# keyber/Single-Image-Super-Resolution

Hardware: AMD Instinct MI355X
Metric: HR patches/sec (x2 generator fwd+bwd, LR 96x96 -> SR 192x192) (higher is better)
Workload: dtype f32; 1 GPU; SRGAN x2 generator (16 blocks, 64 features, spectral norm) fwd+bwd+Adam with bicubic LR degradation and pixel-MSE x10, per-GPU batch 16 HR 192x192 patches (LR 96x96 -> SR 192x192): the north star's headline. BASELINE.json's metric string "96^2 crops, x4" is configs.cfg3 of this line. Single build: fp32.; per_gpu_batch=16, hr=192, lr=96, parallelism=dp1, hip_graph=True

## Files before the change

include/sisr_hip.h:

```cpp
#ifndef SISR_HIP_H
#define SISR_HIP_H

#include <stdint.h>

#ifdef __cplusplus
extern "C" {
#endif

#define SISR_E_BADARG (-1)
#define SISR_E_TOOBIG (-2)
#define SISR_E_UNSUPPORTED (-3)

enum {
    SISR_PRO_NONE = 0,
    SISR_PRO_ACT = 1,
    SISR_PRO_AFFINE_ACT = 2,
    SISR_PRO_BNBWD = 3,
    SISR_PRO_BNACT_BWD = 4,
    SISR_PRO_ACT_BWD = 5,
    SISR_PRO_TANH_BWD = 6,
    SISR_PRO_RES_AFFINE = 7
};
enum { SISR_X_NHWC = 0, SISR_X_NCHW = 1, SISR_X_NHWC_UNSHUFFLE2 = 2 };
enum { SISR_Y_NHWC = 0, SISR_Y_NCHW = 1, SISR_Y_NHWC_SHUFFLE2 = 2 };
// ... 67 lines not shown

typedef struct SisrWgradDeepPlan {
    int32_t enabled;
    int32_t TH, TW, tiles_x, tiles_q, n_tiles;
    int32_t PR;
    int32_t IW, IH_max;
    int32_t IWd, IHd_max;
    int32_t NPOS_max;
    int32_t XP_max;
    int32_t NITX, NITD;
    int32_t n_pb, tiles_per_pb;
    int32_t n_cib, n_cob;
    int32_t lds_bytes;
    int32_t slab_bf16;
    int32_t batch_first_wg;
    uint32_t m_tiles_x, m_tw, m_ho, m_pr, m_iw, m_iwd;
} SisrWgradDeepPlan;

typedef struct SisrWgradDesc {
    const float *x1, *x2, *pa, *pb, *pd, *ps, *pt;
    const float *g1, *g2, *qa, *qb, *qd, *qs, *qt;
    float *slab;
    float *bias_slab;
    int32_t N, H, W, Cin, Ho, Wo, Cout;
    int32_t KH, KW, stride, pad_y, pad_x;
    int32_t x_mode, pro_mode;
    const float *pro_slope_p;
    float pro_slope;
    int32_t g_mode, gpro_mode;
    const float *gpro_slope_p;
    float gpro_slope;
    int32_t TH, TW, TN, tiles_y, tiles_x, n_groups, n_tiles;
    int32_t CK, PS, KROWP, n_chunk, CoutPad;
    int32_t NJ, NP, NT, TSTEP, TVALID;
    int32_t grid_x, n_slabs, slab_elems, lds_bytes;
    uint32_t m_tiles_x, m_tiles_y, m_iw, m_twp, m_kw;
    int32_t x_bf16, g_bf16;
    int32_t mfma_split;
    int64_t slab_stride;
    SisrWgradDeepPlan deep;
} SisrWgradDesc;

int sisr_wgrad_plan(SisrWgradDesc *d, int32_t max_pixel_blocks);
int sisr_conv2d_plan_bf16(SisrConvDesc *d);
int sisr_conv2d_bf16(const SisrConvDesc *d, void *stream);
int sisr_conv2d_deep_plan(SisrConvDesc *d, int32_t target_wg, int32_t prefer_bn, int32_t classes);
int sisr_conv2d_deep_eligible(const SisrConvDesc *d);
int sisr_conv2d_trunk_eligible(const SisrConvDesc *d);
int sisr_conv2d_bf16_parts(const SisrConvDesc *d);
int sisr_conv2d_trunk_f32_eligible(const SisrConvDesc *d);
int sisr_conv2d_f32_parts(const SisrConvDesc *d);
int sisr_conv2d_f32_bnb_parts(const SisrConvDesc *d);
int sisr_conv2d_thin_eligible(const SisrConvDesc *d);
int sisr_conv2d_toimage_eligible(const SisrConvDesc *d);
int sisr_conv2d_toimage_f32_eligible(const SisrConvDesc *d);
int sisr_wgrad_plan_bf16(SisrWgradDesc *d, int32_t max_pixel_blocks);
int sisr_wgrad_deep_plan(SisrWgradDesc *d, int32_t target_wg);
int sisr_wgrad_deep_eligible(const SisrWgradDesc *d);
int sisr_wgrad_deep_batch(const SisrWgradDesc *table_host, const SisrWgradDesc *table_dev, int32_t n, void *stream);
int sisr_wgrad_trunk_batch_arg_bytes(void);
int sisr_wgrad_trunk_batch_args(const SisrWgradDesc *descs, int32_t n, void *args_host);
int sisr_wgrad_trunk_batch(const SisrWgradDesc *descs, const void *args_dev, int32_t n, int32_t wgs_per_layer, void *stream);
int sisr_wgrad_trunk_f32_batch_arg_bytes(void);
int sisr_wgrad_trunk_f32_batch_args(const SisrWgradDesc *descs, int32_t n, void *args_host);
int sisr_wgrad_trunk_f32_batch(const SisrWgradDesc *descs, const void *args_dev, int32_t n, int32_t wgs_per_layer, void *stream);
int sisr_conv2d_wgrad_bf16(const SisrWgradDesc *d, void *stream);
int sisr_wgrad_trunk_eligible(const SisrWgradDesc *d);
int sisr_wgrad_bf16_slabs(const SisrWgradDesc *d);
int sisr_wgrad_trunk_f32_eligible(const SisrWgradDesc *d);
int sisr_wgrad_f32_slabs(const SisrWgradDesc *d);
int sisr_wgrad_thin_eligible(const SisrWgradDesc *d);
int sisr_wgrad_toimage_eligible(const SisrWgradDesc *d);
int sisr_wgrad_toimage_f32_eligible(const SisrWgradDesc *d);
int sisr_conv2d_wgrad_f32(const SisrWgradDesc *d, void *stream);
int sisr_slab_reduce_f32(const float *slab, float *out, int32_t n_slabs, int64_t elems, int64_t lead_bf16, void *stream);
int sisr_slab_reduce_multi(const void *const *slabs, void *const *outs, const int32_t *n_slabs, const int64_t *elems,
                           const int64_t *lead_bf16, int32_t n_jobs, void *stream);
int64_t sisr_wgrad_bf16_slab_lead(const SisrWgradDesc *d);

enum SisrRoute {
    SISR_ROUTE_GENERIC = 0,
    SISR_ROUTE_DEEP = 1,
    SISR_ROUTE_TOIMAGE = 2,
    SISR_ROUTE_TRUNK = 3,
    SISR_ROUTE_THIN = 4
};
int32_t sisr_conv2d_bf16_route(const SisrConvDesc *d);
int32_t sisr_conv2d_f32_route(const SisrConvDesc *d);
int32_t sisr_wgrad_bf16_route(const SisrWgradDesc *d);
int32_t sisr_wgrad_f32_route(const SisrWgradDesc *d);

enum {
    SISR_WIMG_F32 = 0,
    SISR_WIMG_BF16 = 1,
    SISR_WIMG_DEEP = 2
};
typedef struct SisrWeightImage {
    void   *dst;
    int32_t format;
    int32_t transposed;
    int32_t KH, KW;
    int32_t R0y, Sy, R0x, Sx;
    int32_t CK, PS, KROWP, n_chunk, CoutPad;
    int32_t extra;
} SisrWeightImage;
#define SISR_WLDS_WORDS (2 * 2 * 9 * 32 * 36)
#define SISR_WEIGHT_IMAGES 5

typedef struct SisrWeightDesc {
    const float *w_orig;
    float *u, *v;
    float *u_used, *v_used;
    float *sigma;
    float *sn_work;
    int32_t Cout, Cin, KH, KW;
    int32_t training;
    int32_t shuffle2;
    int32_t wdp_scaled;
    SisrWeightImage img[SISR_WEIGHT_IMAGES];
} SisrWeightDesc;
int64_t sisr_weight_image_bytes(const SisrWeightImage *img);

int sisr_weights_prepare(const SisrWeightDesc *table_dev, int32_t n, int32_t max_rows, int32_t max_cols,
                         void *stream);
// ... 161 lines not shown
```

single-image-super-resolution_amd/_lib.py:

```python
import ctypes as C
import os
import subprocess

_HERE = os.path.dirname(os.path.abspath(__file__))
CSRC = os.path.join(_HERE, 'csrc')
LIB_PATH = os.environ.get('SISR_LIB') or os.path.join(CSRC, 'libsisr_hip.so')

PRO_NONE, PRO_ACT, PRO_AFFINE_ACT, PRO_BNBWD, PRO_BNACT_BWD, PRO_ACT_BWD, PRO_TANH_BWD, PRO_RES_AFFINE = range(8)
X_NHWC, X_NCHW, X_UNSHUFFLE2 = range(3)
Y_NHWC, Y_NCHW, Y_SHUFFLE2 = range(3)
EPI_NONE, EPI_TANH = range(2)
ROUTE_GENERIC, ROUTE_DEEP, ROUTE_TOIMAGE, ROUTE_TRUNK, ROUTE_THIN = range(5)

_f = C.c_void_p
_i32 = C.c_int32
_i64 = C.c_int64
_f32 = C.c_float


class ConvPlan(C.Structure):
    _fields_ = [(n, _i32) for n in (
        'TH', 'TW', 'TN', 'tiles_y', 'tiles_x', 'n_groups', 'n_tiles', 'CK', 'PS', 'KROWP', 'n_chunk',
        'CoutPad', 'msub', 'nsub', 'lds_bytes', 'wpk_elems', 'variant')] + [
        (n, C.c_uint32) for n in ('m_tiles_x', 'm_thw', 'm_tw', 'm_iw', 'm_wrow')]
# ... 46 lines not shown

WIMG_F32, WIMG_BF16, WIMG_DEEP = range(3)
WEIGHT_IMAGES = 5


class WeightImage(C.Structure):
    _fields_ = [('dst', _f)] + [(n, _i32) for n in ('format', 'transposed', 'KH', 'KW', 'R0y', 'Sy', 'R0x', 'Sx',
                                                    'CK', 'PS', 'KROWP', 'n_chunk', 'CoutPad', 'extra')]


class WeightDesc(C.Structure):
    _fields_ = ([(n, _f) for n in ('w_orig', 'u', 'v', 'u_used', 'v_used', 'sigma', 'sn_work')] +
                [(n, _i32) for n in ('Cout', 'Cin', 'KH', 'KW', 'training', 'shuffle2', 'wdp_scaled')] +
                [('img', WeightImage * WEIGHT_IMAGES)])


class WeightGradDesc(C.Structure):
    _fields_ = ([(n, _f) for n in ('dwpk', 'w_orig', 'u_used', 'v_used', 'sigma', 'grad', 'dbias_pk',
                                   'grad_bias')] +
                [(n, _i32) for n in ('Cout', 'Cin', 'KH', 'KW', 'shuffle2', 'CK', 'PS', 'KROWP', 'n_chunk',
                                     'CoutPad', 'layout')])


class AdamDesc(C.Structure):
    _fields_ = [('p', _f), ('m', _f), ('v', _f), ('g', _f), ('numel', _i64), ('block_start', _i64)]


class EmaDesc(C.Structure):
    _fields_ = [('ema', _f), ('src', _f), ('numel', _i64), ('block_start', _i64), ('mode', _i32), ('pad', _i32)]


class BnBwdDesc(C.Structure):
    _fields_ = ([(n, _f) for n in ('dy', 'x', 'scale', 'shift', 'mean', 'invstd', 'gamma', 'work',
                                   'qa', 'qb', 'qd', 'dgamma', 'dbeta', 'dslope')] +
                [('P', _i64), ('C', _i32), ('act_mode', _i32), ('slope_p', _f), ('slope', _f32),
                 ('grid', _i32), ('dy_bf16', _i32), ('x_bf16', _i32)])


_SIGS = {
    'sisr_conv2d_plan': [C.POINTER(ConvDesc)],
    'sisr_conv2d_f32': [C.POINTER(ConvDesc), _f],
    'sisr_wgrad_plan': [C.POINTER(WgradDesc), _i32],
    'sisr_conv2d_wgrad_f32': [C.POINTER(WgradDesc), _f],
    'sisr_conv2d_plan_bf16': [C.POINTER(ConvDesc)],
    'sisr_conv2d_bf16': [C.POINTER(ConvDesc), _f],
    'sisr_conv2d_deep_plan': [C.POINTER(ConvDesc), _i32, _i32, _i32],
    'sisr_conv2d_deep_eligible': [C.POINTER(ConvDesc)],
    'sisr_conv2d_trunk_eligible': [C.POINTER(ConvDesc)],
    'sisr_conv2d_bf16_parts': [C.POINTER(ConvDesc)],
    'sisr_conv2d_trunk_f32_eligible': [C.POINTER(ConvDesc)],
    'sisr_conv2d_f32_parts': [C.POINTER(ConvDesc)],
    'sisr_conv2d_f32_bnb_parts': [C.POINTER(ConvDesc)],
    'sisr_conv2d_thin_eligible': [C.POINTER(ConvDesc)],
    'sisr_conv2d_toimage_eligible': [C.POINTER(ConvDesc)],
    'sisr_conv2d_toimage_f32_eligible': [C.POINTER(ConvDesc)],
    'sisr_wgrad_trunk_eligible': [C.POINTER(WgradDesc)],
    'sisr_wgrad_bf16_slabs': [C.POINTER(WgradDesc)],
    'sisr_wgrad_trunk_f32_eligible': [C.POINTER(WgradDesc)],
    'sisr_wgrad_f32_slabs': [C.POINTER(WgradDesc)],
    'sisr_wgrad_thin_eligible': [C.POINTER(WgradDesc)],
    'sisr_wgrad_toimage_eligible': [C.POINTER(WgradDesc)],
    'sisr_wgrad_toimage_f32_eligible': [C.POINTER(WgradDesc)],
    'sisr_wgrad_plan_bf16': [C.POINTER(WgradDesc), _i32],
    'sisr_wgrad_deep_plan': [C.POINTER(WgradDesc), _i32],
    'sisr_wgrad_deep_eligible': [C.POINTER(WgradDesc)],
    'sisr_wgrad_deep_batch': [C.POINTER(WgradDesc), _f, _i32, _f],
    'sisr_wgrad_trunk_batch_arg_bytes': [],
    'sisr_wgrad_trunk_batch_args': [C.POINTER(WgradDesc), _i32, _f],
    'sisr_wgrad_trunk_batch': [C.POINTER(WgradDesc), _f, _i32, _i32, _f],
    'sisr_wgrad_trunk_f32_batch_arg_bytes': [],
    'sisr_wgrad_trunk_f32_batch_args': [C.POINTER(WgradDesc), _i32, _f],
    'sisr_wgrad_trunk_f32_batch': [C.POINTER(WgradDesc), _f, _i32, _i32, _f],
    'sisr_conv2d_wgrad_bf16': [C.POINTER(WgradDesc), _f],
    'sisr_tr16_selftest': [_f, _f],
    'sisr_slab_reduce_f32': [_f, _f, _i32, _i64, _i64, _f],
    'sisr_slab_reduce_multi': [_f, _f, _f, _f, _f, _i32, _f],
    'sisr_wgrad_bf16_slab_lead': [C.POINTER(WgradDesc)],
    'sisr_conv2d_bf16_route': [C.POINTER(ConvDesc)],
    'sisr_conv2d_f32_route': [C.POINTER(ConvDesc)],
    'sisr_wgrad_bf16_route': [C.POINTER(WgradDesc)],
    'sisr_wgrad_f32_route': [C.POINTER(WgradDesc)],
    'sisr_weights_prepare': [_f, _i32, _i32, _i32, _f],
    'sisr_weights_sn': [_f, _i32, _i32, _i32, _f],
    'sisr_weights_pack': [_f, _i32, _i32, _i32, _f],
    'sisr_weights_pack_deep': [_f, _i32, _i32, _i32, _f],
    'sisr_weight_image_bytes': [C.POINTER(WeightImage)],
    'sisr_weights_grad': [_f, _i32, _f, _i32, _f],
    'sisr_weights_grad_fast': [_f, _i32, _f, _i32, _i32, _f],
    'sisr_weights_grad_tiles': [C.POINTER(WeightGradDesc)],
    'sisr_bn_finalize': [_f, _f, _i32, _i32, _f, _f, _f, _f, _f32, _f32, _f, _f, _f, _f, _f],
    'sisr_bn_eval_consts': [_f, _f, _f, _f, _f32, _i32, _f, _f, _f],
    'sisr_bn_bwd_plan': [C.POINTER(BnBwdDesc)],
    'sisr_bn_bwd': [C.POINTER(BnBwdDesc), _f],
    'sisr_bn_bwd_finalize': [C.POINTER(BnBwdDesc), _f],
    'sisr_bn_bwd_finalize_slab': [C.POINTER(BnBwdDesc), _f, _f, _i32, _i64, _i64, _f],
    'sisr_eltwise_res_affine': [_f, _f, _f32, _f, _f, _f, _f, _i64, _i32, _i32, _f],
    'sisr_prelu_slope_grad': [_f, _f, _i64, _f, _f, _i32, _f],
    'sisr_add': [_f, _f, _f, _i64, _i32, _f],
    'sisr_adam_blocks': [_i64],
    'sisr_adam_step': [_f, _i32, _i64] + [C.c_double] * 7 + [_f],
    'sisr_adam_norm_ws_doubles': [_i64],
    'sisr_adam_grad_sumsq': [_f, _i32, _i64, _f, _f],
    'sisr_adam_prepare': [_f, _i32, _f, _i32, C.c_double, C.c_double, _f, _i64, C.c_double, _i32, _i32, _f, _f, _f],
    'sisr_adam_step_dev': [_f, _i32, _i64, _f, _f] + [C.c_double] * 4 + [_f],
    'sisr_ema_prepare': [_f, C.c_double, C.c_double, _f, _f, _f],
    'sisr_ema_update': [_f, _i32, _i64, _f, _f],
    'sisr_ema_swap': [_f, _i32, _i64, _f],
    'sisr_nhwc_to_nchw': [_f, _f, _f, _f, _f32, _f, _i64, _i32, _i32, _i32, _i32, _i32, _f],
    'sisr_nchw_to_nhwc': [_f, _i64, _f, _i32, _i32, _i32, _i32, _i32, _f],
    'sisr_nchw_grad_to_nhwc4': [_f, _f, _f, _i32, _i32, _i32, _i32, _i32, _f],
    'sisr_maxpool2_fwd': [_f, _f, _i32, _i32, _i32, _i32, _i32, _f],
    'sisr_maxpool2_relu_bwd': [_f, _f, _f, _i32, _i32, _i32, _i32, _i32, _f],
    'sisr_add_relu_masked': [_f, _f, _f, _f, _i64, _i32, _f],
# ... 83 lines not shown
```

single-image-super-resolution_amd/csrc/conv_fwd.hip:

```cpp
#include "sisr_dev.h"

#include <algorithm>
#include <cstring>

template <int MSUB, int NSUB, int KU>
__device__ __forceinline__ void conv_kblock(const float* const (&ap)[MSUB], const float* const (&bp)[NSUB], int k0,
                                            f32x16 (&acc)[MSUB][NSUB]) {
    float a[KU][MSUB], b[KU][NSUB];
#pragma unroll
    for (int u = 0; u < KU; ++u) {
#pragma unroll
        for (int ms = 0; ms < MSUB; ++ms) a[u][ms] = ap[ms][k0 + 2 * u];
#pragma unroll
        for (int ns = 0; ns < NSUB; ++ns) b[u][ns] = bp[ns][k0 + 2 * u];
    }
#pragma unroll
    for (int u = 0; u < KU; ++u)
#pragma unroll
        for (int ms = 0; ms < MSUB; ++ms)
#pragma unroll
            for (int ns = 0; ns < NSUB; ++ns) acc[ms][ns] = mfma32(a[u][ms], b[u][ns], acc[ms][ns]);
    __builtin_amdgcn_sched_group_barrier(0x100, KU * (MSUB + NSUB), 0);
    __builtin_amdgcn_sched_group_barrier(0x008, KU * MSUB * NSUB, 0);
}
// ... 333 lines not shown
            p = cand[pick];
            best_lds = cand_lds[pick];
            best_score = 1.0;
        }
    }
    if (best_score < 0) return SISR_E_TOOBIG;
    p.n_chunk = (d->Cin + p.CK - 1) / p.CK;
    p.n_tiles = p.tiles_y * p.tiles_x * p.n_groups;
    p.lds_bytes = best_lds;
    p.wpk_elems = p.n_chunk * d->KH * p.CoutPad * p.KROWP;
    return 0;
}

template <int MSUB, int NSUB, int TAG>
static int launch_conv(const SisrConvDesc* d, hipStream_t st) {
    const dim3 grid(d->plan.n_tiles, d->plan.CoutPad / (NSUB * 32));
    return sisr_launch<conv_mfma_f32_kernel<MSUB, NSUB, TAG>>(grid, dim3(SISR_BLOCK), d->plan.lds_bytes, SISR_LDS_BASE_DEFAULT, st, *d);
}

extern "C" int32_t sisr_conv2d_f32_route(const SisrConvDesc* d) {
    if (!d) return SISR_E_BADARG;
    if (sisr_conv2d_trunk_f32_eligible(d)) return SISR_ROUTE_TRUNK;
    if (sisr_conv2d_thin_eligible(d)) return SISR_ROUTE_THIN;
    return sisr_conv2d_toimage_f32_eligible(d) ? SISR_ROUTE_TOIMAGE : SISR_ROUTE_GENERIC;
}

extern "C" int sisr_conv2d_f32_parts(const SisrConvDesc* d) {
    if (!d) return SISR_E_BADARG;
    return sisr_conv2d_f32_route(d) == SISR_ROUTE_TRUNK ? sisr_conv2d_trunk_f32_streams(d) : d->plan.n_tiles;
}

extern "C" int sisr_conv2d_f32_bnb_parts(const SisrConvDesc* d) {
    if (!d) return SISR_E_BADARG;
    const bool takes = sisr_conv2d_f32_route(d) == SISR_ROUTE_TRUNK && sisr_conv2d_trunk_f32_eligible(d) == 2;
    return takes ? 2 * sisr_conv2d_trunk_f32_streams(d) : 0;
}

extern "C" int sisr_conv2d_f32(const SisrConvDesc* d, void* stream) {
    if (d && d->bnb_part && sisr_conv2d_trunk_f32_eligible(d) != 2) return SISR_E_UNSUPPORTED;
    if (!d || !d->x1 || !d->wpk || !d->y) return SISR_E_BADARG;
    if (operand_needs_x2(d->pro_mode) && !d->x2) return SISR_E_BADARG;
    if (d->stat_part && !d->cnt_part) return SISR_E_BADARG;
    if (d->stat_part && d->y_mode != SISR_Y_NHWC) return SISR_E_UNSUPPORTED;
    if (d->y_bf16 && (d->y_mode == SISR_Y_NCHW || d->res || d->epi_act != SISR_EPI_NONE)) return SISR_E_UNSUPPORTED;
    if (d->res && d->res_bf16) return SISR_E_UNSUPPORTED;
    const SisrConvPlan& p = d->plan;
    if (p.n_tiles <= 0 || p.lds_bytes <= 0 || p.lds_bytes > 160 * 1024) return SISR_E_BADARG;
    hipStream_t st = sisr_stream(stream);
    const int32_t route = sisr_conv2d_f32_route(d);
    if (route == SISR_ROUTE_TRUNK) return sisr_conv2d_trunk_f32_launch(d, st);
    if (route == SISR_ROUTE_THIN) return sisr_conv2d_thin_launch(d, st);
    if (route == SISR_ROUTE_TOIMAGE) return sisr_conv2d_toimage_launch(d, st);
    if (d->pro_mode == SISR_PRO_RES_AFFINE) return SISR_E_UNSUPPORTED;
    const bool trunk = d->Cin == 64 && d->Cout == 64 && d->KH == 3 && d->KW == 3 && d->stride == 1;
    if (p.msub == 2 && p.nsub == 2) return trunk ? launch_conv<2, 2, 1>(d, st) : launch_conv<2, 2, 0>(d, st);
    if (p.msub == 2 && p.nsub == 1) return launch_conv<2, 1, 0>(d, st);
    if (p.msub == 1 && p.nsub == 2) return trunk ? launch_conv<1, 2, 1>(d, st) : launch_conv<1, 2, 0>(d, st);
    if (p.msub == 1 && p.nsub == 1) return launch_conv<1, 1, 0>(d, st);
    return SISR_E_BADARG;
}
```

single-image-super-resolution_amd/csrc/conv_wgrad.hip:

```cpp
#include "sisr_dev.h"

#include <algorithm>
#include <cstring>

#define WG_NACC 9

template <int NACC, int KU>
__device__ __forceinline__ void wgrad_kblock(const float* ip, const float* dyp, const int (&aoff)[NACC], int istep,
                                             int dstep, f32x16 (&acc)[NACC]) {
    float a[KU][NACC], b[KU];
#pragma unroll
    for (int u = 0; u < KU; ++u) {
        b[u] = dyp[u * dstep];
#pragma unroll
        for (int i = 0; i < NACC; ++i) a[u][i] = ip[u * istep + aoff[i]];
    }
#pragma unroll
    for (int u = 0; u < KU; ++u)
#pragma unroll
        for (int i = 0; i < NACC; ++i) acc[i] = mfma32(a[u][i], b[u], acc[i]);
    __builtin_amdgcn_sched_group_barrier(0x100, KU * (NACC + 1), 0);
    __builtin_amdgcn_sched_group_barrier(0x008, KU * NACC, 0);
}

// ... 186 lines not shown
            if (score > best + 1e-9) {
                best = score;
                d->TH = TH; d->TW = TW; d->TN = TN; d->tiles_y = ty; d->tiles_x = tx; d->n_groups = ngr;
                d->lds_bytes = lds;
            }
        }
    }
    if (best < 0) return SISR_E_TOOBIG;
    d->n_tiles = d->tiles_y * d->tiles_x * d->n_groups;
    const int per_pixel_block = d->n_chunk * (d->CoutPad / DSTR);
    int gx = std::max(1, max_pixel_blocks / per_pixel_block);
    d->grid_x = std::min(gx, d->n_tiles);
    d->n_slabs = d->grid_x;
    d->slab_elems = d->n_chunk * d->KH * d->KROWP * d->CoutPad;
    d->slab_stride = d->slab_elems;
    return 0;
}

template <int NACC>
static int launch_wgrad(const SisrWgradDesc* d, hipStream_t st) {
    const dim3 grid(d->grid_x, d->n_chunk * (d->CoutPad / (d->NJ * 32)));
    return sisr_launch<wgrad_mfma_f32_kernel<NACC>>(grid, dim3(SISR_BLOCK), d->lds_bytes, SISR_LDS_BASE_DEFAULT, st, *d);
}

extern "C" int32_t sisr_wgrad_f32_route(const SisrWgradDesc* d) {
    if (!d) return SISR_E_BADARG;
    if (sisr_wgrad_trunk_f32_eligible(d)) return SISR_ROUTE_TRUNK;
    if (sisr_wgrad_thin_eligible(d)) return SISR_ROUTE_THIN;
    return sisr_wgrad_toimage_f32_eligible(d) ? SISR_ROUTE_TOIMAGE : SISR_ROUTE_GENERIC;
}

extern "C" int sisr_wgrad_f32_slabs(const SisrWgradDesc* d) {
    if (!d) return SISR_E_BADARG;
    switch (sisr_wgrad_f32_route(d)) {
        case SISR_ROUTE_TRUNK: return sisr_wgrad_trunk_f32_slabs(d);
        case SISR_ROUTE_THIN: return sisr_wgrad_thin_slabs(d);
        case SISR_ROUTE_TOIMAGE: return sisr_wgrad_toimage_slabs(d);
        default: return d->n_slabs;
    }
}

extern "C" int sisr_conv2d_wgrad_f32(const SisrWgradDesc* d, void* stream) {
    if (!d || !d->x1 || !d->g1 || !d->slab) return SISR_E_BADARG;
    if (operand_needs_x2(d->pro_mode) && !d->x2) return SISR_E_BADARG;
    if (operand_needs_x2(d->gpro_mode) && !d->g2) return SISR_E_BADARG;
    if (d->slab_stride < d->slab_elems) return SISR_E_BADARG;
    if (d->grid_x <= 0 || d->lds_bytes <= 0 || d->lds_bytes > 160 * 1024 || d->KH * d->NT > WG_NACC)
        return SISR_E_BADARG;
    hipStream_t st = sisr_stream(stream);
    const int32_t route = sisr_wgrad_f32_route(d);
    if (route == SISR_ROUTE_TRUNK) return sisr_wgrad_trunk_f32_launch(d, st);
    if (route == SISR_ROUTE_THIN) return sisr_wgrad_thin_launch(d, st);
    if (route == SISR_ROUTE_TOIMAGE) return sisr_wgrad_toimage_f32_launch(d, st);
    switch (d->KH * d->NT) {
        case 1: return launch_wgrad<1>(d, st);
        case 2: return launch_wgrad<2>(d, st);
        case 3: return launch_wgrad<3>(d, st);
        case 4: return launch_wgrad<4>(d, st);
        case 5: return launch_wgrad<5>(d, st);
        case 6: return launch_wgrad<6>(d, st);
        case 7: return launch_wgrad<7>(d, st);
        case 8: return launch_wgrad<8>(d, st);
        case 9: return launch_wgrad<9>(d, st);
    }
    return SISR_E_UNSUPPORTED;
}

extern "C" int sisr_slab_reduce_f32(const float* slab, float* out, int32_t n_slabs, int64_t elems, int64_t lead_bf16,
                                    void* stream) {
    if (!slab || !out || n_slabs <= 0 || elems <= 0) return SISR_E_BADARG;
    if ((elems & 3) || (lead_bf16 & 3) || lead_bf16 < 0 || lead_bf16 > elems) return SISR_E_BADARG;
    const int blocks = (int)((elems / 4 + SR_COLS - 1) / SR_COLS);
    hipLaunchKernelGGL(slab_reduce_kernel, dim3(blocks), dim3(SISR_BLOCK), 0, sisr_stream(stream),
                       slab, out, n_slabs, elems, lead_bf16);
    SISR_CHECK_LAUNCH();
    return 0;
}

extern "C" int sisr_slab_reduce_multi(const void* const* slabs, void* const* outs, const int32_t* n_slabs, const int64_t* elems,
                                      const int64_t* leads, int32_t n_jobs, void* stream) {
    if (!slabs || !outs || !n_slabs || !elems || !leads || n_jobs <= 0) return SISR_E_BADARG;
    for (int i0 = 0; i0 < n_jobs; i0 += SR_MAX_JOBS) {
        SlabJobs j;
        std::memset(&j, 0, sizeof(j));
        j.n = std::min(SR_MAX_JOBS, n_jobs - i0);
        int blocks = 0;
        for (int k = 0; k < j.n; ++k) {
            const int i = i0 + k;
            if (!slabs[i] || !outs[i] || n_slabs[i] <= 0 || elems[i] <= 0) return SISR_E_BADARG;
            if ((elems[i] & 3) || (leads[i] & 3) || leads[i] < 0 || leads[i] > elems[i]) return SISR_E_BADARG;
            j.slab[k] = static_cast<const float*>(slabs[i]); j.out[k] = static_cast<float*>(outs[i]);
            j.n_slabs[k] = n_slabs[i]; j.elems[k] = elems[i]; j.lead[k] = leads[i];
            j.first_block[k] = blocks;
            const int cols = n_slabs[i] <= SR_SPLITS ? SR_FEW_COLS : SR_COLS;
            blocks += (int)((elems[i] / 4 + cols - 1) / cols);
        }
        j.first_block[j.n] = blocks;
        hipLaunchKernelGGL(slab_reduce_multi_kernel, dim3(blocks), dim3(SISR_BLOCK), 0, sisr_stream(stream), j);
        SISR_CHECK_LAUNCH();
    }
    return 0;
}
```

single-image-super-resolution_amd/csrc/sisr_host.h:

```cpp
#pragma once
#include <hip/hip_runtime.h>
#include <cstdlib>
#include "../../include/sisr_hip.h"

#define SISR_CHECK_LAUNCH()                          \
    do {                                             \
        hipError_t e__ = hipGetLastError();          \
        if (e__ != hipSuccess) return (int)e__;      \
    } while (0)

static inline hipStream_t sisr_stream(void* s) { return reinterpret_cast<hipStream_t>(s); }

static inline bool sisr_switch_off(const char* name) {
    const char* e = getenv(name);
    return e && e[0] == '0';
}

#define SISR_MAX_DEVICES 64
int sisr_device_index();
int sisr_cu_slots();
static inline int sisr_equal_shares(int total, int slots, int* rounds_out = nullptr) {
    if (slots < 1) slots = 1;
    const int rounds = (total + slots - 1) / slots;
    if (rounds_out) *rounds_out = rounds;
    return (total + rounds - 1) / rounds;
}
struct SisrLdsCap { int v[SISR_MAX_DEVICES]; };
#define SISR_LDS_BASE_DEFAULT (64 * 1024)
static inline int sisr_raise_lds_cap(SisrLdsCap& cap, const void* fn, int bytes, int base) {
    int& cur = cap.v[sisr_device_index()];
    if (cur < base) cur = base;
    if (bytes <= cur) return 0;
    hipError_t e = hipFuncSetAttribute(fn, hipFuncAttributeMaxDynamicSharedMemorySize, bytes);
    if (e != hipSuccess) return (int)e;
    cur = bytes;
    return 0;
}
template <auto K, typename... Args>
static int sisr_launch(dim3 grid, dim3 block, int lds, int lds_base, hipStream_t st, const Args&... args) {
    static SisrLdsCap cap;
    if (int e = sisr_raise_lds_cap(cap, reinterpret_cast<const void*>(K), lds, lds_base)) return e;
    hipLaunchKernelGGL(K, grid, block, lds, st, args...);
    SISR_CHECK_LAUNCH();
    return 0;
}

int sisr_conv2d_trunk_launch(const SisrConvDesc* d, hipStream_t st);
int sisr_conv2d_trunk_grid(const SisrConvDesc* d);
int sisr_conv2d_trunk_f32_launch(const SisrConvDesc* d, hipStream_t st);
int sisr_conv2d_trunk_f32_streams(const SisrConvDesc* d);
int sisr_conv2d_thin_launch(const SisrConvDesc* d, hipStream_t st);
int sisr_conv2d_toimage_launch(const SisrConvDesc* d, hipStream_t st);
int sisr_conv2d_deep_launch(const SisrConvDesc* d, hipStream_t st);
int sisr_conv2d_deep_parts(const SisrConvDesc* d);
int sisr_wgrad_trunk_launch(const SisrWgradDesc* d, hipStream_t st);
int sisr_wgrad_trunk_slabs(const SisrWgradDesc* d);
int sisr_wgrad_trunk_f32_launch(const SisrWgradDesc* d, hipStream_t st);
int sisr_wgrad_trunk_f32_slabs(const SisrWgradDesc* d);
int sisr_wgrad_thin_launch(const SisrWgradDesc* d, hipStream_t st);
int sisr_wgrad_thin_slabs(const SisrWgradDesc* d);
int sisr_wgrad_toimage_launch(const SisrWgradDesc* d, hipStream_t st);
int sisr_wgrad_toimage_f32_launch(const SisrWgradDesc* d, hipStream_t st);
int sisr_wgrad_toimage_slabs(const SisrWgradDesc* d);
int sisr_wgrad_deep_launch(const SisrWgradDesc* d, hipStream_t st);
```

Measured before the change: 1489 HR patches/s.

## Add dedicated f32 MFMA kernels for 3-channel image conv forward and wgrad

Adds specialized persistent kernels for convolutions whose input is the 3-channel NCHW image: a forward kernel for the 9x9 head conv and the 3x3 tanh-backward conv, and a weight-gradient kernel for the 9x9 head. The forward kernel keeps weights in registers, double-buffers halo tiles in LDS with prefetch, and stores NHWC output. The wgrad kernel accumulates per-workgroup partials into slabs, fusing the leaky-ReLU backward and the bias sum. The aim is to replace the generic f32 conv paths, which handle the thin Cin=3 case inefficiently, at the cost of two new code paths with strict eligibility checks.

```diff
diff --git a/include/sisr_hip.h b/include/sisr_hip.h
--- a/include/sisr_hip.h
+++ b/include/sisr_hip.h
@@ -143,6 +143,7 @@
 int sisr_conv2d_f32_parts(const SisrConvDesc *d);
 int sisr_conv2d_f32_bnb_parts(const SisrConvDesc *d);
 int sisr_conv2d_thin_eligible(const SisrConvDesc *d);
+int sisr_conv2d_image_f32_eligible(const SisrConvDesc *d);
 int sisr_conv2d_toimage_eligible(const SisrConvDesc *d);
 int sisr_conv2d_toimage_f32_eligible(const SisrConvDesc *d);
 int sisr_wgrad_plan_bf16(SisrWgradDesc *d, int32_t max_pixel_blocks);
@@ -161,6 +162,7 @@
 int sisr_wgrad_trunk_f32_eligible(const SisrWgradDesc *d);
 int sisr_wgrad_f32_slabs(const SisrWgradDesc *d);
 int sisr_wgrad_thin_eligible(const SisrWgradDesc *d);
+int sisr_wgrad_image_f32_eligible(const SisrWgradDesc *d);
 int sisr_wgrad_toimage_eligible(const SisrWgradDesc *d);
 int sisr_wgrad_toimage_f32_eligible(const SisrWgradDesc *d);
 int sisr_conv2d_wgrad_f32(const SisrWgradDesc *d, void *stream);
diff --git a/single-image-super-resolution_amd/_lib.py b/single-image-super-resolution_amd/_lib.py
--- a/single-image-super-resolution_amd/_lib.py
+++ b/single-image-super-resolution_amd/_lib.py
@@ -122,6 +122,7 @@
     'sisr_conv2d_f32_parts': [C.POINTER(ConvDesc)],
     'sisr_conv2d_f32_bnb_parts': [C.POINTER(ConvDesc)],
     'sisr_conv2d_thin_eligible': [C.POINTER(ConvDesc)],
+    'sisr_conv2d_image_f32_eligible': [C.POINTER(ConvDesc)],
     'sisr_conv2d_toimage_eligible': [C.POINTER(ConvDesc)],
     'sisr_conv2d_toimage_f32_eligible': [C.POINTER(ConvDesc)],
     'sisr_wgrad_trunk_eligible': [C.POINTER(WgradDesc)],
@@ -129,6 +130,7 @@
     'sisr_wgrad_trunk_f32_eligible': [C.POINTER(WgradDesc)],
     'sisr_wgrad_f32_slabs': [C.POINTER(WgradDesc)],
     'sisr_wgrad_thin_eligible': [C.POINTER(WgradDesc)],
+    'sisr_wgrad_image_f32_eligible': [C.POINTER(WgradDesc)],
     'sisr_wgrad_toimage_eligible': [C.POINTER(WgradDesc)],
     'sisr_wgrad_toimage_f32_eligible': [C.POINTER(WgradDesc)],
     'sisr_wgrad_plan_bf16': [C.POINTER(WgradDesc), _i32],
diff --git a/single-image-super-resolution_amd/csrc/conv_fwd.hip b/single-image-super-resolution_amd/csrc/conv_fwd.hip
--- a/single-image-super-resolution_amd/csrc/conv_fwd.hip
+++ b/single-image-super-resolution_amd/csrc/conv_fwd.hip
@@ -409,6 +409,7 @@
     if (route == SISR_ROUTE_THIN) return sisr_conv2d_thin_launch(d, st);
     if (route == SISR_ROUTE_TOIMAGE) return sisr_conv2d_toimage_launch(d, st);
     if (d->pro_mode == SISR_PRO_RES_AFFINE) return SISR_E_UNSUPPORTED;
+    if (sisr_conv2d_image_f32_eligible(d)) return sisr_conv2d_image_f32_launch(d, st);
     const bool trunk = d->Cin == 64 && d->Cout == 64 && d->KH == 3 && d->KW == 3 && d->stride == 1;
     if (p.msub == 2 && p.nsub == 2) return trunk ? launch_conv<2, 2, 1>(d, st) : launch_conv<2, 2, 0>(d, st);
     if (p.msub == 2 && p.nsub == 1) return launch_conv<2, 1, 0>(d, st);
diff --git a/single-image-super-resolution_amd/csrc/conv_image_f32.hip b/single-image-super-resolution_amd/csrc/conv_image_f32.hip
--- /dev/null
+++ b/single-image-super-resolution_amd/csrc/conv_image_f32.hip
@@ -0,0 +1,185 @@
+#include "sisr_dev.h"
+
+#include <algorithm>
+#include <cstdlib>
+
+typedef unsigned img_u32x4 __attribute__((ext_vector_type(4)));
+
+#define IMG_TW 16
+#define IMG_IW 48
+
+template <int KS> struct ImageGeom {
+    static constexpr int MT = KS == 9 ? 2 : 4;
+    static constexpr int TH = 4 * MT;
+    static constexpr int ROW = KS * 3;
+    static constexpr int K = KS * ROW;
+    static constexpr int NS = (K + 1) / 2;
+    static constexpr int IH = TH + KS - 1, IWV = IMG_TW + KS - 1;
+    static constexpr int HALO = IH * IMG_IW * 3 + 4;
+    static constexpr int ITEMS = (IH * IWV + 255) / 256;
+    static constexpr int KROWP = (ROW + 3) / 4 * 4;
+    static constexpr int WELEMS = KS * 64 * KROWP;
+    static constexpr int LDS = (WELEMS > 2 * HALO ? WELEMS : 2 * HALO) * 4;
+};
+
+struct ImageArgs {
+    const float *x1, *x2, *wpk, *bias;
+    float* y;
+    int N, H, W;
+    int tiles_x, per_img, total, rounds;
+};
+
+template <int KS, bool TANHB>
+__global__ void __launch_bounds__(256, 1) conv_image_f32_kernel(const ImageArgs a) {
+    typedef ImageGeom<KS> G;
+    constexpr int MT = G::MT, TH = G::TH, ROW = G::ROW, K = G::K, NS = G::NS, IH = G::IH, IWV = G::IWV, HALO = G::HALO,
+                  ITEMS = G::ITEMS, KROWP = G::KROWP, PAD = (KS - 1) / 2, PITCH = IMG_IW * 3;
+    __shared__ __attribute__((aligned(16))) float lds[G::LDS / 4];
+    const int tid = threadIdx.x, lane = tid & 63, wave = tid >> 6;
+    const int l31 = lane & 31, kk = lane >> 5, h = wave & 1, g = wave >> 1;
+    const int prow = l31 >> 4, px = l31 & 15;
+
+    {
+        const f32x4* src = reinterpret_cast<const f32x4*>(a.wpk);
+        f32x4* dst = reinterpret_cast<f32x4*>(lds);
+        for (int i = tid; i < G::WELEMS / 4; i += 256) dst[i] = src[i];
+    }
+    __syncthreads();
+    float wv[NS];
+    {
+        const float* wa = lds + (32 * h + l31) * KROWP + kk;
+        const float* wb = lds + (32 * h + l31) * KROWP + kk * (64 * KROWP - (ROW - 1));
+#pragma unroll
+        for (int s = 0; s < NS; ++s) {
+            const int k0 = 2 * s, ky = k0 / ROW, j = k0 - ky * ROW;
+            if (k0 + 1 >= K) wv[s] = kk ? 0.f : wa[ky * 64 * KROWP + j];
+            else wv[s] = (j == ROW - 1 ? wb : wa)[ky * 64 * KROWP + j];
+        }
+    }
+    float bv[16];
+#pragma unroll
+    for (int i = 0; i < 16; ++i) bv[i] = 0.f;
+    if (a.bias != nullptr) {
+#pragma unroll
+        for (int i = 0; i < 16; ++i) bv[i] = a.bias[32 * h + mfma_row(i, lane)];
+    }
+    __syncthreads();
+    for (int i = tid; i < 2 * HALO; i += 256) lds[i] = 0.f;
+    __syncthreads();
+
+    const unsigned plane = (unsigned)(a.H * a.W);
+    const unsigned xbytes = (unsigned)a.N * 3u * plane * 4u;
+    const __amdgpu_buffer_rsrc_t rx = sisr_rsrc(a.x1, xbytes), rx2 = sisr_rsrc(TANHB ? a.x2 : a.x1, xbytes);
+    int hy[ITEMS], hx[ITEMS], rel[ITEMS];
+#pragma unroll
+    for (int k = 0; k < ITEMS; ++k) {
+        const int id = tid + 256 * k;
+        hy[k] = id / IWV;
+        hx[k] = id - hy[k] * IWV;
+        rel[k] = ((hy[k] - PAD) * a.W + hx[k] - PAD) * 4;
+    }
+    const int t_first = blockIdx.x * a.rounds, t_end = min(t_first + a.rounds, a.total);
+    float sv[ITEMS][3], sw[ITEMS][3];
+    auto issue = [&](int T) {
+        const int n = T / a.per_img, r = T - n * a.per_img;
+        const int ty = r / a.tiles_x, tx = r - ty * a.tiles_x;
+        const int origin = ((n * 3 * a.H + ty * TH) * a.W + tx * IMG_TW) * 4;
+        const int live = T < t_end;
+#pragma unroll
+        for (int k = 0; k < ITEMS; ++k) {
+            const int y = ty * TH - PAD + hy[k], x = tx * IMG_TW - PAD + hx[k];
+            const int ok = live & (int)(hy[k] < IH) & (int)((unsigned)y < (unsigned)a.H) & (int)((unsigned)x < (unsigned)a.W);
+            const unsigned base = (unsigned)(origin + rel[k]), dead = ok ? 0u : 0x80000000u;
+#pragma unroll
+            for (int c = 0; c < 3; ++c) {
+                const unsigned voff = (base + (unsigned)c * plane * 4u) | dead;
+                sv[k][c] = __builtin_bit_cast(float, __builtin_amdgcn_raw_buffer_load_b32(rx, voff, 0, 0));
+                if (TANHB) sw[k][c] = __builtin_bit_cast(float, __builtin_amdgcn_raw_buffer_load_b32(rx2, voff, 0, 0));
+            }
+        }
+    };
+    auto commit = [&](float* buf) {
+#pragma unroll
+        for (int k = 0; k < ITEMS; ++k) {
+            float* p = buf + (hy[k] < IH ? (hy[k] * IMG_IW + hx[k]) * 3 : HALO - 4);
+#pragma unroll
+            for (int c = 0; c < 3; ++c) p[c] = TANHB ? sv[k][c] * (1.f - sw[k][c] * sw[k][c]) : sv[k][c];
+        }
+    };
+
+    const unsigned ybytes = (unsigned)a.N * plane * 256u;
+    const __amdgpu_buffer_rsrc_t ry = sisr_rsrc(a.y, ybytes);
+    const int b_pix = ((2 * MT * g + prow) * IMG_IW + px) * 3;
+    const int b_a = b_pix + kk, b_b = b_pix + kk * (PITCH - (ROW - 1));
+
+    int T = t_first;
+    issue(T);
+    commit(lds);
+    __syncthreads();
+    issue(T + 1);
+    int cur = 0;
+    for (; T < t_end; ++T, cur ^= 1) {
+        f32x16 acc[MT];
+#pragma unroll
+        for (int mt = 0; mt < MT; ++mt)
+#pragma unroll
+            for (int i = 0; i < 16; ++i) acc[mt][i] = 0.f;
+        const float* ia = lds + cur * HALO + b_a;
+        const float* ib = lds + cur * HALO + b_b;
+#pragma unroll
+        for (int s = 0; s < NS; ++s) {
+            const int k0 = 2 * s, ky = k0 / ROW, j = k0 - ky * ROW;
+            const float* p = ((j == ROW - 1 && k0 + 1 < K) ? ib : ia) + ky * PITCH + j;
+#pragma unroll
+            for (int mt = 0; mt < MT; ++mt) acc[mt] = mfma32(wv[s], p[2 * mt * PITCH], acc[mt]);
+        }
+        __builtin_amdgcn_sched_barrier(0);
+        commit(lds + (cur ^ 1) * HALO);
+        issue(T + 2);
+        const int n = T / a.per_img, r = T - n * a.per_img;
+        const int ty = r / a.tiles_x, tx = r - ty * a.tiles_x;
+#pragma unroll
+        for (int mt = 0; mt < MT; ++mt) {
+            const int oy = ty * TH + 2 * MT * g + 2 * mt + prow, ox = tx * IMG_TW + px;
+            const unsigned pix = ((unsigned)(n * a.H + oy) * (unsigned)a.W + (unsigned)ox) * 256u;
+#pragma unroll
+            for (int q = 0; q < 4; ++q) {
+                const f32x4 o = {acc[mt][4 * q] + bv[4 * q], acc[mt][4 * q + 1] + bv[4 * q + 1], acc[mt][4 * q + 2] + bv[4 * q + 2],
+                                 acc[mt][4 * q + 3] + bv[4 * q + 3]};
+                __builtin_amdgcn_raw_buffer_store_b128(__builtin_bit_cast(img_u32x4, o), ry,
+                                                       pix + (unsigned)(32 * h + 8 * q + 4 * kk) * 4u, 0, 0);
+            }
+        }
+        __syncthreads();
+    }
+}
+
+extern "C" int sisr_conv2d_image_f32_eligible(const SisrConvDesc* d) {
+    if (sisr_switch_off("SISR_IMAGE_F32") || !d) return 0;
+    if (d->x_mode != SISR_X_NCHW || d->x_bf16 || d->Cin != 3 || d->Cout != 64 || d->plan.CoutPad != 64) return 0;
+    if ((d->KH != 9 && d->KH != 3) || d->KW != d->KH || d->stride != 1 || d->pad_y != (d->KH - 1) / 2 || d->pad_x != d->pad_y) return 0;
+    if (d->pro_mode != (d->KH == 9 ? SISR_PRO_NONE : SISR_PRO_TANH_BWD)) return 0;
+    if (d->y_mode != SISR_Y_NHWC || d->y_bf16 || d->res || d->stat_part || d->bnb_part || d->epi_act != SISR_EPI_NONE) return 0;
+    if (d->y_sy != 1 || d->y_sx != 1 || d->y_oy != 0 || d->y_ox != 0 || d->y_H != d->Ho || d->y_W != d->Wo) return 0;
+    const int th = d->KH == 9 ? ImageGeom<9>::TH : ImageGeom<3>::TH;
+    if (d->Ho != d->H || d->Wo != d->W || (d->H % th) || (d->W % IMG_TW)) return 0;
+    if (d->plan.n_chunk != 1 || d->plan.PS != 3 || d->plan.KROWP != (d->KH == 9 ? ImageGeom<9>::KROWP : ImageGeom<3>::KROWP)) return 0;
+    if ((int64_t)d->N * d->H * d->W * 256 >= (1ll << 31)) return 0;
+    return 1;
+}
+
+int sisr_conv2d_image_f32_launch(const SisrConvDesc* d, hipStream_t st) {
+    const bool tanhb = d->pro_mode == SISR_PRO_TANH_BWD;
+    if (tanhb && !d->x2) return SISR_E_BADARG;
+    ImageArgs a;
+    a.x1 = d->x1; a.x2 = d->x2; a.wpk = d->wpk; a.bias = d->bias; a.y = d->y;
+    a.N = d->N; a.H = d->H; a.W = d->W;
+    a.tiles_x = d->W / IMG_TW;
+    a.per_img = a.tiles_x * (d->H / (d->KH == 9 ? ImageGeom<9>::TH : ImageGeom<3>::TH));
+    a.total = a.per_img * d->N;
+    const dim3 grid(sisr_equal_shares(a.total, sisr_cu_slots(), &a.rounds)), block(256);
+    if (d->KH == 9) hipLaunchKernelGGL((conv_image_f32_kernel<9, false>), grid, block, 0, st, a);
+    else hipLaunchKernelGGL((conv_image_f32_kernel<3, true>), grid, block, 0, st, a);
+    SISR_CHECK_LAUNCH();
+    return 0;
+}
diff --git a/single-image-super-resolution_amd/csrc/conv_wgrad.hip b/single-image-super-resolution_amd/csrc/conv_wgrad.hip
--- a/single-image-super-resolution_amd/csrc/conv_wgrad.hip
+++ b/single-image-super-resolution_amd/csrc/conv_wgrad.hip
@@ -262,6 +262,7 @@
     if (route == SISR_ROUTE_TRUNK) return sisr_wgrad_trunk_f32_launch(d, st);
     if (route == SISR_ROUTE_THIN) return sisr_wgrad_thin_launch(d, st);
     if (route == SISR_ROUTE_TOIMAGE) return sisr_wgrad_toimage_f32_launch(d, st);
+    if (sisr_wgrad_image_f32_eligible(d)) return sisr_wgrad_image_f32_launch(d, st);
     switch (d->KH * d->NT) {
         case 1: return launch_wgrad<1>(d, st);
         case 2: return launch_wgrad<2>(d, st);
diff --git a/single-image-super-resolution_amd/csrc/sisr_host.h b/single-image-super-resolution_amd/csrc/sisr_host.h
--- a/single-image-super-resolution_amd/csrc/sisr_host.h
+++ b/single-image-super-resolution_amd/csrc/sisr_host.h
@@ -50,6 +50,7 @@
 int sisr_conv2d_trunk_f32_launch(const SisrConvDesc* d, hipStream_t st);
 int sisr_conv2d_trunk_f32_streams(const SisrConvDesc* d);
 int sisr_conv2d_thin_launch(const SisrConvDesc* d, hipStream_t st);
+int sisr_conv2d_image_f32_launch(const SisrConvDesc* d, hipStream_t st);
 int sisr_conv2d_toimage_launch(const SisrConvDesc* d, hipStream_t st);
 int sisr_conv2d_deep_launch(const SisrConvDesc* d, hipStream_t st);
 int sisr_conv2d_deep_parts(const SisrConvDesc* d);
@@ -59,6 +60,7 @@
 int sisr_wgrad_trunk_f32_slabs(const SisrWgradDesc* d);
 int sisr_wgrad_thin_launch(const SisrWgradDesc* d, hipStream_t st);
 int sisr_wgrad_thin_slabs(const SisrWgradDesc* d);
+int sisr_wgrad_image_f32_launch(const SisrWgradDesc* d, hipStream_t st);
 int sisr_wgrad_toimage_launch(const SisrWgradDesc* d, hipStream_t st);
 int sisr_wgrad_toimage_f32_launch(const SisrWgradDesc* d, hipStream_t st);
 int sisr_wgrad_toimage_slabs(const SisrWgradDesc* d);
diff --git a/single-image-super-resolution_amd/csrc/wgrad_image_f32.hip b/single-image-super-resolution_amd/csrc/wgrad_image_f32.hip
--- /dev/null
+++ b/single-image-super-resolution_amd/csrc/wgrad_image_f32.hip
@@ -0,0 +1,202 @@
+#include "sisr_dev.h"
+
+#include <algorithm>
+#include <cstdlib>
+
+#define WIF_TH 4
+#define WIF_TW 16
+#define WIF_IH (WIF_TH + 8)
+#define WIF_IWV (WIF_TW + 8)
+#define WIF_IW 41
+#define WIF_PITCH (3 * WIF_IW)
+#define WIF_XH (WIF_IH * WIF_PITCH + 4)
+#define WIF_DY (WIF_TH * WIF_TW * 64)
+#define WIF_XITEMS ((WIF_IH * WIF_IWV + 255) / 256)
+#define WIF_GITEMS (WIF_DY / 4 / 256)
+#define WIF_NCOL 243
+#define WIF_PSTR 257
+#define WIF_SLAB (9 * 28 * 64)
+#define WIF_LDS_FLOATS (64 * WIF_PSTR + 256 * 4)
+
+struct WImageF32Args {
+    const float *x, *g1, *g2;
+    float *slab, *bias_slab;
+    const float* slope_p;
+    float slope;
+    int N, H, W;
+    int tiles_x, per_img, total, rounds, n_slabs;
+    long long slab_stride;
+};
+
+template <bool ACTB>
+__global__ void __launch_bounds__(256, 1) wgrad_image_f32_kernel(const WImageF32Args a) {
+    extern __shared__ __attribute__((aligned(16))) float lds[];
+    float* dys = lds;
+    float* xhs = lds + 2 * WIF_DY;
+    const int tid = threadIdx.x, lane = tid & 63, wave = tid >> 6, l31 = lane & 31, kk = lane >> 5;
+    const float slope = a.slope_p ? a.slope_p[0] : a.slope;
+
+    for (int row = blockIdx.x + gridDim.x; row < a.n_slabs; row += gridDim.x) {
+        f32x4* z = reinterpret_cast<f32x4*>(a.slab + (long long)row * a.slab_stride);
+        for (int i = tid; i < WIF_SLAB / 4; i += 256) z[i] = f32x4{0.f, 0.f, 0.f, 0.f};
+        if (a.bias_slab != nullptr && tid < 64) a.bias_slab[(long long)row * a.slab_stride + tid] = 0.f;
+    }
+    for (int i = tid; i < 2 * WIF_XH; i += 256) xhs[i] = 0.f;
+    __syncthreads();
+
+    int boff[2];
+#pragma unroll
+    for (int nb = 0; nb < 2; ++nb) {
+        const int n = 32 * (2 * wave + nb) + l31, nn = n < WIF_NCOL ? n : n - 32;
+        const int ky = nn / 27;
+        boff[nb] = ky * WIF_PITCH + (nn - 27 * ky) + 3 * kk;
+    }
+
+    const unsigned plane = (unsigned)(a.H * a.W);
+    const __amdgpu_buffer_rsrc_t rx = sisr_rsrc(a.x, (unsigned)a.N * 3u * plane * 4u);
+    const __amdgpu_buffer_rsrc_t rg = sisr_rsrc(a.g1, (unsigned)a.N * plane * 256u),
+                                 rp = sisr_rsrc(ACTB ? a.g2 : a.g1, (unsigned)a.N * plane * 256u);
+    int hy[WIF_XITEMS], hx[WIF_XITEMS];
+#pragma unroll
+    for (int k = 0; k < WIF_XITEMS; ++k) {
+        const int id = tid + 256 * k;
+        hy[k] = id / WIF_IWV;
+        hx[k] = id - hy[k] * WIF_IWV;
+    }
+    const int t_first = blockIdx.x * a.rounds, t_end = min(t_first + a.rounds, a.total);
+    float sx[WIF_XITEMS][3];
+    f32x4 sg[WIF_GITEMS], sp[WIF_GITEMS];
+    f32x4 bsum = {0.f, 0.f, 0.f, 0.f};
+
+    auto issue = [&](int T) {
+        const int n = T / a.per_img, r = T - n * a.per_img;
+        const int ty = r / a.tiles_x, tx = r - ty * a.tiles_x;
+        const int live = T < t_end;
+#pragma unroll
+        for (int k = 0; k < WIF_XITEMS; ++k) {
+            const int Y = ty * WIF_TH - 4 + hy[k], X = tx * WIF_TW - 4 + hx[k];
+            const int ok = live & (int)(hy[k] < WIF_IH) & (int)((unsigned)Y < (unsigned)a.H) & (int)((unsigned)X < (unsigned)a.W);
+            const unsigned base = (unsigned)(((n * 3 * a.H + Y) * a.W + X) * 4), dead = ok ? 0u : 0x80000000u;
+#pragma unroll
+            for (int c = 0; c < 3; ++c)
+                sx[k][c] = __builtin_bit_cast(float, __builtin_amdgcn_raw_buffer_load_b32(rx, (base + (unsigned)c * plane * 4u) | dead, 0, 0));
+        }
+        const int origin = ((n * a.H + ty * WIF_TH) * a.W + tx * WIF_TW) * 256;
+        const unsigned dead_tile = live ? 0u : 0x80000000u;
+#pragma unroll
+        for (int i = 0; i < WIF_GITEMS; ++i) {
+            const int grp = tid + 256 * i, p = grp >> 4, c4 = grp & 15;
+            const unsigned voff = (unsigned)(origin + ((p >> 4) * a.W + (p & 15)) * 256 + c4 * 16) | dead_tile;
+            sg[i] = __builtin_bit_cast(f32x4, __builtin_amdgcn_raw_buffer_load_b128(rg, voff, 0, 0));
+            if (ACTB) sp[i] = __builtin_bit_cast(f32x4, __builtin_amdgcn_raw_buffer_load_b128(rp, voff, 0, 0));
+        }
+    };
+    auto commit = [&](int buf) {
+        float* xh = xhs + buf * WIF_XH;
+#pragma unroll
+        for (int k = 0; k < WIF_XITEMS; ++k) {
+            float* p = xh + (hy[k] < WIF_IH ? (hy[k] * WIF_IW + hx[k]) * 3 : WIF_XH - 4);
+#pragma unroll
+            for (int c = 0; c < 3; ++c) p[c] = sx[k][c];
+        }
+        float* dy = dys + buf * WIF_DY;
+#pragma unroll
+        for (int i = 0; i < WIF_GITEMS; ++i) {
+            f32x4 v = sg[i];
+            if (ACTB) {
+#pragma unroll
+                for (int j = 0; j < 4; ++j) v[j] = sp[i][j] > 0.f ? v[j] : slope * v[j];
+            }
+            bsum += v;
+            *reinterpret_cast<f32x4*>(dy + (tid + 256 * i) * 4) = v;
+        }
+    };
+
+    f32x16 acc[2][2];
+#pragma unroll
+    for (int mh = 0; mh < 2; ++mh)
+#pragma unroll
+        for (int nb = 0; nb < 2; ++nb)
+#pragma unroll
+            for (int i = 0; i < 16; ++i) acc[mh][nb][i] = 0.f;
+
+    int T = t_first;
+    issue(T);
+    commit(0);
+    __syncthreads();
+    issue(T + 1);
+    int cur = 0;
+    for (; T < t_end; ++T, cur ^= 1) {
+        const float* ap = dys + cur * WIF_DY + kk * 64 + l31;
+        const float* bp0 = xhs + cur * WIF_XH + boff[0];
+        const float* bp1 = xhs + cur * WIF_XH + boff[1];
+#pragma unroll
+        for (int py = 0; py < WIF_TH; ++py)
+#pragma unroll
+            for (int s = 0; s < WIF_TW / 2; ++s) {
+                const float a0 = ap[(py * WIF_TW + 2 * s) * 64], a1 = ap[(py * WIF_TW + 2 * s) * 64 + 32];
+                const float b0 = bp0[py * WIF_PITCH + 6 * s], b1 = bp1[py * WIF_PITCH + 6 * s];
+                acc[0][0] = mfma32(a0, b0, acc[0][0]);
+                acc[0][1] = mfma32(a0, b1, acc[0][1]);
+                acc[1][0] = mfma32(a1, b0, acc[1][0]);
+                acc[1][1] = mfma32(a1, b1, acc[1][1]);
+            }
+        __builtin_amdgcn_sched_barrier(0);
+        commit(cur ^ 1);
+        issue(T + 2);
+        __syncthreads();
+    }
+
+    float* part = lds;
+    float* bred = lds + 64 * WIF_PSTR;
+#pragma unroll
+    for (int mh = 0; mh < 2; ++mh)
+#pragma unroll
+        for (int nb = 0; nb < 2; ++nb)
+#pragma unroll
+            for (int i = 0; i < 16; ++i)
+                part[(32 * mh + mfma_row(i, lane)) * WIF_PSTR + 32 * (2 * wave + nb) + l31] = acc[mh][nb][i];
+    *reinterpret_cast<f32x4*>(bred + 4 * tid) = bsum;
+    __syncthreads();
+    float* sl = a.slab + (long long)blockIdx.x * a.slab_stride;
+    for (int idx = tid; idx < WIF_SLAB; idx += 256) {
+        const int co = idx & 63, t = idx >> 6, ky = t / 28, krow = t - 28 * ky;
+        sl[idx] = krow < 27 ? part[co * WIF_PSTR + 27 * ky + krow] : 0.f;
+    }
+    if (a.bias_slab != nullptr && tid < 64) {
+        float s = 0.f;
+        for (int i = 0; i < 16; ++i) s += bred[4 * (16 * i + (tid >> 2)) + (tid & 3)];
+        a.bias_slab[(long long)blockIdx.x * a.slab_stride + tid] = s;
+    }
+}
+
+extern "C" int sisr_wgrad_image_f32_eligible(const SisrWgradDesc* d) {
+    if (sisr_switch_off("SISR_IMAGE_F32") || !d) return 0;
+    if (d->KH != 9 || d->KW != 9 || d->stride != 1 || d->pad_y != 4 || d->pad_x != 4) return 0;
+    if (d->Cin != 3 || d->Cout != 64 || d->CoutPad != 64 || d->n_chunk != 1 || d->PS != 3 || d->KROWP != 28 || d->slab_elems != WIF_SLAB) return 0;
+    if (d->x_mode != SISR_X_NCHW || d->x_bf16 || d->pro_mode != SISR_PRO_NONE) return 0;
+    if (d->g_mode != SISR_X_NHWC || d->g_bf16 || (d->gpro_mode != SISR_PRO_NONE && d->gpro_mode != SISR_PRO_ACT_BWD)) return 0;
+    if (d->Ho != d->H || d->Wo != d->W || (d->H % WIF_TH) || (d->W % WIF_TW)) return 0;
+    if (d->n_slabs < 1 || (d->slab_stride & 3)) return 0;
+    if ((int64_t)d->N * d->H * d->W * 256 >= (1ll << 31)) return 0;
+    return 1;
+}
+
+int sisr_wgrad_image_f32_launch(const SisrWgradDesc* d, hipStream_t st) {
+    const bool actb = d->gpro_mode == SISR_PRO_ACT_BWD;
+    if (actb && !d->g2) return SISR_E_BADARG;
+    WImageF32Args a;
+    a.x = d->x1; a.g1 = d->g1; a.g2 = d->g2; a.slab = d->slab; a.bias_slab = d->bias_slab;
+    a.slope_p = d->gpro_slope_p; a.slope = d->gpro_slope;
+    a.N = d->N; a.H = d->H; a.W = d->W;
+    a.tiles_x = d->W / WIF_TW;
+    a.per_img = a.tiles_x * (d->H / WIF_TH);
+    a.total = a.per_img * d->N;
+    a.n_slabs = d->n_slabs;
+    a.slab_stride = d->slab_stride;
+    const int grid = sisr_equal_shares(a.total, std::min(sisr_cu_slots(), (int)d->n_slabs), &a.rounds);
+    constexpr int lds_bytes = WIF_LDS_FLOATS * 4;
+    static_assert(WIF_LDS_FLOATS >= 2 * WIF_DY + 2 * WIF_XH, "the epilogue image is the larger use of LDS");
+    if (actb) return sisr_launch<wgrad_image_f32_kernel<true>>(dim3(grid), dim3(256), lds_bytes, 0, st, a);
+    return sisr_launch<wgrad_image_f32_kernel<false>>(dim3(grid), dim3(256), lds_bytes, 0, st, a);
+}
```

New measurement: 1501 HR patches/s (median of 6 runs). About the same (+0.8%).
